# Glaciohound/Chimera-ST

Measured on AMD Instinct MI355X. Metric: train utterances/sec, MuST-C EN-DE s2t_transformer_m, 1/2/4/8 MI355X, higher is better.
Workload: dtype bf16

## Files before the change

chimera-st_amd/csrc/layernorm.hip:

```cpp
#include "cst_common.h"

namespace {

constexpr int LN_MAXV = 4;
constexpr int LN_WAVES = 4;

template <typename T> struct Raw8;
template <> struct Raw8<bf16_t> {
  u32x4 r;
  __device__ __forceinline__ void load(const bf16_t* p) { r = *reinterpret_cast<const u32x4*>(p); }
  __device__ __forceinline__ void unpack(float (&v)[8]) const {
#pragma unroll
    for (int i = 0; i < 4; ++i) { v[2 * i] = __uint_as_float(r[i] << 16); v[2 * i + 1] = __uint_as_float(r[i] & 0xffff0000u); }
  }
};
template <> struct Raw8<float> {
  float f[8];
  __device__ __forceinline__ void load(const float* p) { load8(p, f); }
  __device__ __forceinline__ void unpack(float (&v)[8]) const {
#pragma unroll
    for (int i = 0; i < 8; ++i) v[i] = f[i];
  }
};

// ... 54 lines not shown
#pragma unroll
    for (int i = 0; i < NV; ++i)
      if (lane + 64 * i < nvec) {
#pragma unroll
        for (int e = 0; e < 8; ++e) { const float d = v[i][e] - mu; q += d * d; }
      }
    const float rs = rsqrtf(wave_sum(q) / (float)cols + eps);
#pragma unroll
    for (int i = 0; i < NV; ++i) {
      const int vi = lane + 64 * i;
      if (vi < nvec) {
        float g[8], b[8], o[8];
        gq[i].unpack(g);
        bq[i].unpack(b);
#pragma unroll
        for (int e = 0; e < 8; ++e) o[e] = (v[i][e] - mu) * rs * g[e] + b[e];
        store8(y + row * cols + vi * 8, o);
      }
    }
    if (lane == 0) { mean[row] = mu; rstd[row] = rs; }
  }
}

template <typename T, int NV>
__global__ __launch_bounds__(LN_WAVES * 64, (NV <= 2 ? 4 : 2)) void ln_bwd_kernel(const T* dy, const T* s, const T* gamma, const float* mean,
                                                              const float* rstd, const T* dres, T* dx, float* part,
                                                              int64_t rows, int cols, uint32_t* tile_live, uint32_t epoch) {
  __shared__ float red[LN_WAVES][64 * 8];
  const int lane = threadIdx.x & 63, wave = threadIdx.x >> 6;
  const int nvec = cols / 8;
  float dg[NV][8], db[NV][8], gm[NV][8];
#pragma unroll
  for (int i = 0; i < NV; ++i) {
#pragma unroll
    for (int e = 0; e < 8; ++e) { dg[i][e] = 0.0f; db[i][e] = 0.0f; gm[i][e] = 0.0f; }
    if (lane + 64 * i < nvec) load8(gamma + (lane + 64 * i) * 8, gm[i]);
  }
  for (int64_t row = (int64_t)blockIdx.x * LN_WAVES + wave; row < rows; row += (int64_t)gridDim.x * LN_WAVES) {
    const float mu = mean[row], rs = rstd[row];
    Raw8<T> rd[NV], rx[NV];
    float s1 = 0.0f, s2 = 0.0f;
#pragma unroll
    for (int i = 0; i < NV; ++i) {
      const int vi = lane + 64 * i;
      if (vi < nvec) {
        rd[i].load(dy + row * cols + vi * 8);
        rx[i].load(s + row * cols + vi * 8);
        float d[8], xs[8];
        rd[i].unpack(d);
        rx[i].unpack(xs);
#pragma unroll
        for (int e = 0; e < 8; ++e) {
          const float xh = (xs[e] - mu) * rs;
          const float g = d[e] * gm[i][e];
          s1 += g;
          s2 += g * xh;
          dg[i][e] += d[e] * xh;
          db[i][e] += d[e];
        }
      }
    }
    s1 = wave_sum(s1) / (float)cols;
    s2 = wave_sum(s2) / (float)cols;
    bool nz = false;
#pragma unroll
    for (int i = 0; i < NV; ++i) {
      const int vi = lane + 64 * i;
      if (vi < nvec) {
        float d[8], xs[8], o[8];
        rd[i].unpack(d);
        rx[i].unpack(xs);
#pragma unroll
        for (int e = 0; e < 8; ++e) o[e] = rs * (d[e] * gm[i][e] - s1 - (xs[e] - mu) * rs * s2);
        if (dres) {
          float r[8];
          load8(dres + row * cols + vi * 8, r);
#pragma unroll
          for (int e = 0; e < 8; ++e) o[e] += r[e];
        }
#pragma unroll
        for (int e = 0; e < 8; ++e) nz |= (o[e] != 0.0f);
        store8(dx + row * cols + vi * 8, o);
      }
    }
    if (tile_live && __builtin_amdgcn_ballot_w64(nz) != 0 && lane == 0) tile_live[row >> 6] = epoch;
  }
  float* pg = part + (int64_t)blockIdx.x * 2 * cols;
  float* pb = pg + cols;
#pragma unroll
  for (int i = 0; i < NV; ++i) {
    for (int pass = 0; pass < 2; ++pass) {
      __syncthreads();
#pragma unroll
      for (int e = 0; e < 8; ++e) red[wave][lane * 8 + e] = pass ? db[i][e] : dg[i][e];
      __syncthreads();
      if (wave == 0 && lane + 64 * i < nvec) {
#pragma unroll
        for (int e = 0; e < 8; ++e) {
          float a = 0.0f;
#pragma unroll
          for (int w = 0; w < LN_WAVES; ++w) a += red[w][lane * 8 + e];
          (pass ? pb : pg)[(lane + 64 * i) * 8 + e] = a;
        }
      }
    }
  }
}

template <typename TO>
__global__ __launch_bounds__(1024) void ln_bwd_reduce_kernel(const float* part, TO* dgamma, TO* dbeta, int nblocks, int cols) {
  __shared__ float ra[64][17], rb[64][17];
  const int cl = threadIdx.x & 15, g = threadIdx.x >> 4;
  const int c = blockIdx.x * 16 + cl;
  float a = 0.0f, b = 0.0f;
  if (c < cols)
    for (int i = g; i < nblocks; i += 64) {
      a += part[(int64_t)i * 2 * cols + c];
      b += part[(int64_t)i * 2 * cols + cols + c];
    }
  ra[g][cl] = a;
  rb[g][cl] = b;
  __syncthreads();
  if (g == 0 && c < cols) {
#pragma unroll 8
    for (int k = 1; k < 64; ++k) { a += ra[k][cl]; b += rb[k][cl]; }
    DT<TO>::st(dgamma + c, a);
    DT<TO>::st(dbeta + c, b);
  }
}

int ln_blocks(int64_t rows, int cap = 1024) {
  int64_t b = cst_ceil_div(rows, LN_WAVES);
  return (int)(b < cap ? b : cap);
}
inline int ln_nv(int64_t cols) { return cols <= 512 ? 1 : (cols <= 1024 ? 2 : 4); }

}

extern "C" int cst_layernorm_fwd(const void* x, const void* res, const void* gamma, const void* beta, void* y,
                                 void* sum_out, float* mean, float* rstd, int64_t rows, int64_t cols, float eps,
                                 int dtype, cst_stream stream) {
  CST_REQUIRE(x && gamma && beta && y && mean && rstd, "cst_layernorm_fwd: null tensor");
  CST_REQUIRE(rows > 0 && cols > 0 && cols % 8 == 0 && cols <= 8 * 64 * LN_MAXV, "cst_layernorm_fwd: cols=%lld must be a multiple of 8 and <= %d", (long long)cols, 8 * 64 * LN_MAXV);
  hipStream_t s = (hipStream_t)stream;
  const double bytes = (double)rows * cols * cst_dtype_size(dtype) * (2.0 + (res ? 1.0 : 0.0) + (sum_out ? 1.0 : 0.0));
  CstProfScope prof(CST_K_LAYERNORM, s, 0.0, bytes);
  dim3 grid(ln_blocks(rows, 2048));
  CST_REQUIRE(dtype == CST_BF16 || dtype == CST_F32, "cst_layernorm_fwd: bad dtype %d", dtype);
#define CST_LNF(T, NVV) hipLaunchKernelGGL((ln_fwd_kernel<T, NVV>), grid, dim3(LN_WAVES * 64), 0, s, (const T*)x, (const T*)res, (const T*)gamma, (const T*)beta, (T*)y, (T*)sum_out, mean, rstd, rows, (int)cols, eps)
#define CST_LNF_NV(T) do { const int nv = ln_nv(cols); if (nv == 1) CST_LNF(T, 1); else if (nv == 2) CST_LNF(T, 2); else CST_LNF(T, 4); } while (0)
  if (dtype == CST_BF16) CST_LNF_NV(bf16_t);
  else CST_LNF_NV(float);
#undef CST_LNF_NV
#undef CST_LNF
  return cst_check_launch("cst_layernorm_fwd");
}

constexpr int LN_BWD_BLOCKS = 1024;
extern "C" int64_t cst_layernorm_bwd_workspace(int64_t rows, int64_t cols) {
  return (int64_t)ln_blocks(rows, LN_BWD_BLOCKS) * 2 * cols * (int64_t)sizeof(float);
}

static int layernorm_bwd_impl(const void* dy, const void* sx, const void* gamma, const float* mean, const float* rstd,
                              const void* dres, void* dx, void* dgamma, void* dbeta, void* workspace, int64_t rows,
                              int64_t cols, int dtype, int grad_dtype, uint32_t* tile_live, uint32_t epoch, cst_stream stream) {
  CST_REQUIRE(dy && sx && gamma && mean && rstd && dx && workspace && ((dgamma != nullptr) == (dbeta != nullptr)), "cst_layernorm_bwd: null tensor");
  CST_REQUIRE(rows > 0 && cols > 0 && cols % 8 == 0 && cols <= 8 * 64 * LN_MAXV, "cst_layernorm_bwd: cols=%lld must be a multiple of 8 and <= %d", (long long)cols, 8 * 64 * LN_MAXV);
  hipStream_t s = (hipStream_t)stream;
  const double bytes = (double)rows * cols * cst_dtype_size(dtype) * (3.0 + (dres ? 1.0 : 0.0));
  CstProfScope prof(CST_K_LAYERNORM, s, 0.0, bytes);
  const int nb = ln_blocks(rows, LN_BWD_BLOCKS);
  CST_REQUIRE(dtype == CST_BF16 || dtype == CST_F32, "cst_layernorm_bwd: bad dtype %d", dtype);
#define CST_LNB(T, NVV) hipLaunchKernelGGL((ln_bwd_kernel<T, NVV>), dim3(nb), dim3(LN_WAVES * 64), 0, s, (const T*)dy, (const T*)sx, (const T*)gamma, mean, rstd, (const T*)dres, (T*)dx, (float*)workspace, rows, (int)cols, tile_live, epoch)
#define CST_LNB_NV(T) do { const int nv = ln_nv(cols); if (nv == 1) CST_LNB(T, 1); else if (nv == 2) CST_LNB(T, 2); else CST_LNB(T, 4); } while (0)
  if (dtype == CST_BF16) CST_LNB_NV(bf16_t);
  else CST_LNB_NV(float);
#undef CST_LNB_NV
#undef CST_LNB
  int rc = cst_check_launch("cst_layernorm_bwd");
  if (rc != CST_OK) return rc;
  CST_REQUIRE(grad_dtype == CST_F32 || grad_dtype == dtype, "cst_layernorm_bwd: grad_dtype must be f32 or dtype");
  if (!dgamma) return rc;
  if (grad_dtype == CST_BF16)
    hipLaunchKernelGGL(ln_bwd_reduce_kernel<bf16_t>, dim3((unsigned)cst_ceil_div(cols, 16)), dim3(1024), 0, s, (const float*)workspace, (bf16_t*)dgamma, (bf16_t*)dbeta, nb, (int)cols);
  else
    hipLaunchKernelGGL(ln_bwd_reduce_kernel<float>, dim3((unsigned)cst_ceil_div(cols, 16)), dim3(1024), 0, s, (const float*)workspace, (float*)dgamma, (float*)dbeta, nb, (int)cols);
  return cst_check_launch("cst_layernorm_bwd reduce");
}

extern "C" int cst_layernorm_bwd(const void* dy, const void* sx, const void* gamma, const float* mean, const float* rstd,
                                 const void* dres, void* dx, void* dgamma, void* dbeta, void* workspace, int64_t rows,
                                 int64_t cols, int dtype, int grad_dtype, cst_stream stream) {
  return layernorm_bwd_impl(dy, sx, gamma, mean, rstd, dres, dx, dgamma, dbeta, workspace, rows, cols, dtype, grad_dtype, nullptr, 0, stream);
}

extern "C" int cst_layernorm_bwd_tiles(const void* dy, const void* sx, const void* gamma, const float* mean, const float* rstd,
                                       const void* dres, void* dx, void* dgamma, void* dbeta, void* workspace, int64_t rows,
                                       int64_t cols, int dtype, int grad_dtype, uint32_t* tile_live, uint32_t epoch, cst_stream stream) {
  CST_REQUIRE(tile_live && epoch != 0, "cst_layernorm_bwd_tiles: tile_live / non-zero epoch required");
  return layernorm_bwd_impl(dy, sx, gamma, mean, rstd, dres, dx, dgamma, dbeta, workspace, rows, cols, dtype, grad_dtype, tile_live, epoch, stream);
}
```

chimera-st_amd/functional.py:

```python
import os as _os
import weakref as _weakref

import torch

from . import kernels as K
from . import lib as L

_ACT = {None: L.ACT_NONE, "none": L.ACT_NONE, "relu": L.ACT_RELU, "gelu": L.ACT_GELU}


def _flat2d(x):
    return x.reshape(-1, x.shape[-1]).contiguous()


def _vec(dtype):
    return 8 if dtype == torch.bfloat16 else 4


def _with_tiles(t, tiles):
    if t.is_contiguous():
        t._cst_live_tiles = (tiles[0], tiles[1], t.data_ptr(), t.numel(), t.shape[-1], t._version)
        if t._base is not None:
            t._base._cst_live_tiles = t._cst_live_tiles
    return t


def _tiles_of(t, rows):
    lt = getattr(t, "_cst_live_tiles", None)
    if lt is None and t._base is not None:
        lt = getattr(t._base, "_cst_live_tiles", None)
    if (lt is None or not t.is_contiguous() or lt[2] != t.data_ptr() or lt[3] != t.numel() or lt[4] != t.shape[-1]
            or lt[5] != t._version or lt[0].numel() != (rows + 63) // 64):
        return None
    return (lt[0], lt[1])


_WT_MIN_ROWS = int(_os.environ.get("CST_WT_MIN_ROWS", 512))


def _want_wt(M, w):
    return (M >= _WT_MIN_ROWS and w.is_cuda and w.dim() == 2 and w.is_contiguous() and w.shape[0] % _vec(w.dtype) == 0
            and w.shape[1] % _vec(w.dtype) == 0 and not _os.environ.get("CST_NO_WT"))


def _wversion(w):
    parts = getattr(w, "_cst_parts", None)
    return w._version if parts is None else sum(p._version for p in parts)


class _WeightTransposes:

    def __init__(self):
        self.entries = {}
        self.tables = {}
        self.refreshes = 0
        self.persistent = {}

# ... 125 lines not shown

def _dx_gemm(dz, w, M, *, use_wt, like, resid=None, dact=L.ACT_NONE, aux_in=None, drop=(0.0, 0), m_live=None):
    n_out, n_in = w.shape
    dx = torch.empty(M, n_in, dtype=like.dtype, device=like.device)
    b, b_kmajor, ldb = (WEIGHT_TRANSPOSES.get(w), 1, n_out) if use_wt else (w, 0, n_in)
    K.gemm(dz, b, dx, M, n_in, n_out, a_kmajor=1, b_kmajor=b_kmajor, lda=n_out, ldb=ldb, ldc=n_in, dact=dact, aux_in=aux_in, ld_aux_in=n_in,
           resid=resid, ld_resid=n_in, split_k=1, drop_p=drop[0], drop_key=drop[1], m_live=m_live)
    return dx


def _dw_gemm(dz, x2, w, bias_obj, M, *, db_in_dw, live, dz_travels_on, allow_slot=True, allow_defer=True):
    n_out, n_in = w.shape
    dw = _grad_out(w) if allow_slot else None
    if dw is None:
        dw = torch.empty(n_out, n_in, dtype=w.dtype, device=w.device)
    db = torch.empty(n_out, dtype=w.dtype, device=w.device) if db_in_dw else None
    may = allow_defer and _may_defer(w, bias_obj if db_in_dw else None)
    big = not may or not K.dw_colsum_is_fused(n_out, n_in, M, w.dtype) or dz_travels_on
    K.side_gemm(big, (dz, x2, live[0] if live is not None else None), dz, x2, dw, n_out, n_in, M, a_kmajor=0, b_kmajor=0, lda=n_out, ldb=n_in,
                ldc=n_in, split_k=-1, k_live=live, colsum=db, defer=may)
    return dw, db


def _drop_grad(dy2, drop, out_dtype, live, *, with_colsum, defer):
    if with_colsum and not _os.environ.get("CST_NO_DROP_COLSUM"):
        return K.dropout_colsum(dy2.contiguous(), drop[0], drop[1], out_dtype, live, defer=defer)
    return K.dropout(dy2.contiguous(), *drop), None


def _linear_backward(ctx, dy, dxp):
    x2, w, z = ctx.saved_tensors
    M, Kd = x2.shape
    Np, N = w.shape[0], ctx.N
    if dy is None:
        return dxp, None, None, None, None, None, None
    dy2 = _flat2d(dy)
    live = _tiles_of(dy, M)
    if Np != N:
        dyp = torch.zeros(M, Np, dtype=dy2.dtype, device=dy2.device)
        dyp[:, :N] = dy2
        dy2 = dyp
    db_fused = None
    want_db = ctx.has_bias and ctx.needs_input_grad[2]
    db_in_dw = want_db and ctx.needs_input_grad[1] and Np % 8 == 0 and not _os.environ.get("CST_NO_GEMM_COLSUM") and K.dw_colsum_is_fused(Np, Kd, M, w.dtype)
    may_b = want_db and Np == N and _may_defer(w, ctx.bias_obj)
    if ctx.drop[0] > 0.0:
        dy2, db_fused = _drop_grad(dy2, ctx.drop, w.dtype, live, defer=may_b,
                                   with_colsum=not db_in_dw and ctx.act == L.ACT_NONE and want_db and Np == N and N % 8 == 0)
    dz = K.act_bwd(dy2, z, ctx.act) if ctx.act != L.ACT_NONE else dy2
    dx = dw = db = dres = None
    if ctx.needs_input_grad[0]:
        dx = _dx_gemm(dz, w, M, use_wt=_want_wt(M, w), like=x2, resid=_flat2d(dxp) if dxp is not None else None,
                      m_live=live).view(ctx.xshape)
        if live is not None and dxp is None:
            dx = _with_tiles(dx, live)
    if ctx.needs_input_grad[1]:
        dw, db = _dw_gemm(dz, x2, w, ctx.bias_obj, M, db_in_dw=db_in_dw, live=live, dz_travels_on=dz.data_ptr() == dy.data_ptr() and ctx.has_resid,
                          allow_slot=Np == N, allow_defer=Np == N)
        dw = dw[:N]
        if db is not None:
            db = db[:N]
    if want_db and db is None:
        db = db_fused if db_fused is not None else K.colsum(dz, w.dtype, live, defer=may_b)[:N]
    if ctx.has_resid and ctx.needs_input_grad[3]:
        dres = dy
    return dx, dw, db, dres, None, None, None


class _LinearPassFn(torch.autograd.Function):

    @staticmethod
    def forward(ctx, x, weight, bias, act, drop_p, drop_key):
        y = _LinearFn.forward(ctx, x, weight, bias, None, act, drop_p, drop_key)
        ctx.set_materialize_grads(False)
        return y, x.view_as(x)

    @staticmethod
    def backward(ctx, dy, dxp):
        g = _linear_backward(ctx, dy, dxp)
        return g[0], g[1], g[2], None, None, None


def linear_pass(x, weight, bias=None, act=None, dropout_p=0.0):
    return _LinearPassFn.apply(x, weight, bias, _ACT[act], *_drop_args(dropout_p))


def linear(x, weight, bias=None, act=None, resid=None, dropout_p=0.0):
    return _LinearFn.apply(x, weight, bias, resid, _ACT[act], *_drop_args(dropout_p))


class _FFNFn(torch.autograd.Function):

    @staticmethod
    def forward(ctx, x, w1, b1, w2, b2, resid, act, p_act, key_act, p_out, key_out):
        x2 = _flat2d(x)
        M, d = x2.shape
        F_ = w1.shape[0]
        dout = w2.shape[0]
        z1 = torch.empty(M, F_, dtype=x.dtype, device=x.device)
        h = torch.empty_like(z1)
        K.gemm(x2, w1, h, M, F_, d, a_kmajor=1, b_kmajor=1, lda=d, ldb=d, ldc=F_, bias=b1, act=act, aux_out=z1, ld_aux_out=F_, split_k=1,
               drop_p=p_act, drop_key=key_act)
        y = torch.empty(M, dout, dtype=x.dtype, device=x.device)
        r2 = _flat2d(resid) if resid is not None else None
        K.gemm(h, w2, y, M, dout, F_, a_kmajor=1, b_kmajor=1, lda=F_, ldb=F_, ldc=dout, bias=b2, resid=r2, ld_resid=dout, split_k=1,
               drop_p=p_out, drop_key=key_out)
        ctx.save_for_backward(x2, w1, w2, z1, h)
        ctx.cfg = (act, b1 is not None, b2 is not None, resid is not None, x.shape)
        ctx.res_is_x = (resid is not None and resid.data_ptr() == x.data_ptr() and resid.shape == x.shape
                        and resid.stride() == x.stride() and dout == d)
        ctx.drop = (p_act, key_act, p_out, key_out)
        ctx.bias_objs = (b1, b2)
        return y.view(*x.shape[:-1], dout)

    @staticmethod
    def backward(ctx, dy):
        x2, w1, w2, z1, h = ctx.saved_tensors
        act, has_b1, has_b2, has_res, xshape = ctx.cfg
        M, d = x2.shape
        F_, dout = w1.shape[0], w2.shape[0]
        dy2 = _flat2d(dy)
        live = _tiles_of(dy, M)
        p_act, key_act, p_out, key_out = ctx.drop
        b1, b2 = ctx.bias_objs
        db2_fused = None
        gcs = not _os.environ.get("CST_NO_GEMM_COLSUM")
        db2_in_dw = gcs and has_b2 and ctx.needs_input_grad[4] and ctx.needs_input_grad[3] and dout % 8 == 0 and K.dw_colsum_is_fused(dout, F_, M, w2.dtype)
        db1_in_dw = gcs and has_b1 and ctx.needs_input_grad[2] and ctx.needs_input_grad[1] and F_ % 8 == 0 and K.dw_colsum_is_fused(F_, d, M, w1.dtype)
        if p_out > 0.0:
            dy2, db2_fused = _drop_grad(dy2, (p_out, key_out), w2.dtype, live, defer=_may_defer(w2, b2),
                                        with_colsum=not db2_in_dw and has_b2 and ctx.needs_input_grad[4] and dout % 8 == 0)
        use_wt = _want_wt(M, w2) and _want_wt(M, w1)
        dz1 = _dx_gemm(dy2, w2, M, use_wt=use_wt, like=dy2, dact=act, aux_in=z1, drop=(p_act, key_act), m_live=live)
        dx = dw1 = db1 = dw2 = db2 = None
        if ctx.needs_input_grad[3]:
            dw2, db2 = _dw_gemm(dy2, h, w2, b2, M, db_in_dw=db2_in_dw, live=live, dz_travels_on=dy2.data_ptr() == dy.data_ptr() and has_res)
        if has_b2 and ctx.needs_input_grad[4] and db2 is None:
            db2 = db2_fused if db2_fused is not None else K.colsum(dy2, w2.dtype, live, defer=_may_defer(w2, b2))
        if ctx.needs_input_grad[0]:
            dx = _dx_gemm(dz1, w1, M, use_wt=use_wt, like=x2, resid=_flat2d(dy) if ctx.res_is_x else None, m_live=live).view(xshape)
        if ctx.needs_input_grad[1]:
            dw1, db1 = _dw_gemm(dz1, x2, w1, b1, M, db_in_dw=db1_in_dw, live=live, dz_travels_on=False)
        if has_b1 and ctx.needs_input_grad[2] and db1 is None:
            db1 = K.colsum(dz1, w1.dtype, live, defer=_may_defer(w1, b1))
        dres = dy if has_res and ctx.needs_input_grad[5] and not (ctx.res_is_x and ctx.needs_input_grad[0]) else None
        return dx, dw1, db1, dw2, db2, dres, None, None, None, None, None


def ffn(x, w1, b1, w2, b2, act, resid=None, activation_dropout_p=0.0, dropout_p=0.0):
    assert _ACT[act] != L.ACT_NONE
    return _FFNFn.apply(x, w1.contiguous(), b1, w2.contiguous(), b2, resid, _ACT[act], *_drop_args(activation_dropout_p), *_drop_args(dropout_p))


class _LayerNormFn(torch.autograd.Function):
    @staticmethod
    def forward(ctx, x, res, gamma, beta, eps):
        x2 = _flat2d(x)
        r2 = _flat2d(res) if res is not None else None
        y, s, mean, rstd = K.layernorm_fwd(x2, r2, gamma, beta, eps, want_sum=True)
        src = s if res is not None else x2
        ctx.save_for_backward(src, gamma, mean, rstd)
        ctx.has_res = res is not None
        ctx.shape = x.shape
        ctx.set_materialize_grads(False)
        if res is not None:
            return y.view(x.shape), s.view(x.shape)
        return y.view(x.shape), None

    @staticmethod
    def backward(ctx, dy, ds):
        src, gamma, mean, rstd = ctx.saved_tensors
        if dy is None:
            return ds, (ds if ctx.has_res else None), None, None, None
        dy2 = _flat2d(dy)
        dres = _flat2d(ds) if ds is not None else None
        dx, dg, db, tiles = K.layernorm_bwd(dy2, src, gamma, mean, rstd, dres, grad_dtype=gamma.dtype, want_tiles=True, defer=_may_defer(gamma))
        dx = _with_tiles(dx.view(ctx.shape), tiles)
        return dx, (dx if ctx.has_res else None), dg, db, None


def layer_norm(x, gamma, beta, eps=1e-5):
    return _LayerNormFn.apply(x, None, gamma, beta, eps)[0]


def add_layer_norm(x, res, gamma, beta, eps=1e-5):
    return _LayerNormFn.apply(x, res, gamma, beta, eps)


class _LayerNormPassFn(torch.autograd.Function):

    @staticmethod
    def forward(ctx, x, gamma, beta, eps):
        x2 = _flat2d(x)
        y, _, mean, rstd = K.layernorm_fwd(x2, None, gamma, beta, eps)
        ctx.save_for_backward(x2, gamma, mean, rstd)
        ctx.shape = x.shape
        ctx.set_materialize_grads(False)
        return y.view(x.shape), x.view_as(x)

    @staticmethod
    def backward(ctx, dy, dxp):
        x2, gamma, mean, rstd = ctx.saved_tensors
        dres = _flat2d(dxp) if dxp is not None else None
        if dy is None:
            return (dxp, None, None, None)
        dx, dg, db = K.layernorm_bwd(_flat2d(dy), x2, gamma, mean, rstd, dres, grad_dtype=gamma.dtype, defer=_may_defer(gamma))
        return dx.view(ctx.shape), dg, db, None


def layer_norm_residual(x, gamma, beta, eps=1e-5):
    return _LayerNormPassFn.apply(x, gamma, beta, eps)


_MASK_CACHE = []


_PAD_TILES = []


def _pad_tiles(u8):
    for src, pt in _PAD_TILES:
        if src is u8:
            return pt
    flat = u8.reshape(-1)
    pad = (-flat.numel()) % 64
    if pad:
        flat = torch.cat([flat, torch.ones(pad, dtype=flat.dtype, device=flat.device)])
    pt = flat.view(-1, 64).amin(dim=1) > 0
    _PAD_TILES.append((u8, pt))
    if len(_PAD_TILES) > 8:
# ... 667 lines not shown
```

chimera-st_amd/kernels.py:

```python
import ctypes
import os

import torch

from . import lib as L

_ws = {}
STATS = {}


def workspace(nbytes: int, device) -> torch.Tensor:
    key = (device.index, L.stream_ptr().value)
    t = _ws.get(key)
    if t is None or t.numel() < nbytes:
        t = torch.empty(max(nbytes, 1 << 20), dtype=torch.uint8, device=device)
        _ws[key] = t
    return t


class _Deferred:

    MAX_BYTES = 32 << 20

    def __init__(self):
# ... 232 lines not shown
def layernorm_bwd(dy, s, gamma, mean, rstd, dres=None, grad_dtype=torch.float32, want_tiles=False, defer=False):
    dy, s = _2d(dy), _2d(s)
    rows, cols = s.shape
    lib = L.load()
    dx = torch.empty_like(s)
    dg = torch.empty(cols, dtype=grad_dtype, device=s.device)
    db = torch.empty(cols, dtype=grad_dtype, device=s.device)
    stamps, epoch = (torch.empty((rows + 63) // 64, dtype=torch.int32, device=s.device), next_epoch()) if want_tiles else (None, 0)

    def launch(ws, pg, pb):
        if want_tiles:
            L.check(lib.cst_layernorm_bwd_tiles(L.ptr(dy), L.ptr(s), L.ptr(gamma), L.ptr(mean), L.ptr(rstd), L.ptr(dres), L.ptr(dx), pg,
                                                pb, L.ptr(ws), rows, cols, L.dtype_code(s.dtype), L.dtype_code(grad_dtype),
                                                L.ptr(stamps), epoch, L.stream_ptr()), "cst_layernorm_bwd_tiles")
        else:
            L.check(lib.cst_layernorm_bwd(L.ptr(dy), L.ptr(s), L.ptr(gamma), L.ptr(mean), L.ptr(rstd), L.ptr(dres), L.ptr(dx), pg,
                                          pb, L.ptr(ws), rows, cols, L.dtype_code(s.dtype), L.dtype_code(grad_dtype), L.stream_ptr()),
                    "cst_layernorm_bwd")

    _two_stage(lib.cst_layernorm_bwd_workspace(rows, cols), (dg, db), defer, launch)
    return (dx, dg, db, (stamps, epoch)) if want_tiles else (dx, dg, db)


def _bhtd_strides(t, layout):
    assert t.stride(-1) == 1
    if layout == "bt":
        return t.stride(0), None, t.stride(1)
    return t.stride(1), None, t.stride(0)


def attn_desc(q, k, v, o, lse, H, D, kpm, causal, scale, layout_q="bt", layout_kv="bt", drop_p=0.0, drop_key=0, kv_len=None, seq=None):
    d = L.AttnDesc()
    d.dtype = L.dtype_code(q.dtype)
    if layout_q == "bt":
        B, Tq = q.shape[0], q.shape[1]
    else:
        Tq, B = q.shape[0], q.shape[1]
    Tk = k.shape[1] if layout_kv == "bt" else k.shape[0]
    if seq is not None:
        assert layout_q == "bt" and layout_kv == "bt" and B == 1 and kpm is None
        assert seq[0].dtype == torch.int32 and seq[0].is_contiguous()
        B, Tq, Tk = seq[0].numel() - 1, int(seq[1]), int(seq[1])
        d.seq_offsets = seq[0].data_ptr()
        STATS["attn_packed"] = STATS.get("attn_packed", 0) + 1
    else:
        d.seq_offsets = None
# ... 468 lines not shown
```

chimera-st_amd/lib.py:

```python
import ctypes
import os

import torch

_HERE = os.path.dirname(os.path.abspath(__file__))
LIB_PATH = os.path.join(_HERE, "libcst_hip.so")
ABI_VERSION = 10

F32, BF16 = 0, 1
ACT_NONE, ACT_RELU, ACT_GELU = 0, 1, 2
BIAS_NONE, BIAS_COL, BIAS_ROW = 0, 1, 2
K_GEMM, K_ATTN_FWD, K_ATTN_BWD, K_LAYERNORM, K_CONV0, K_ELEMENTWISE, K_LOSS, K_OPTIM = range(8)
KERNEL_CLASSES = ["gemm", "attn_fwd", "attn_bwd", "layernorm", "conv0", "elementwise", "loss", "optim"]

c_i64, c_int, c_f, c_p = ctypes.c_int64, ctypes.c_int, ctypes.c_float, ctypes.c_void_p


class GemmDesc(ctypes.Structure):
    _fields_ = [
        ("dtype", c_int), ("c_dtype", c_int), ("a_kmajor", c_int), ("b_kmajor", c_int),
        ("M", c_i64), ("N", c_i64), ("K", c_i64),
        ("A", c_p), ("lda", c_i64), ("a_seg", c_i64), ("a_seg_stride", c_i64),
        ("B", c_p), ("ldb", c_i64), ("b_seg", c_i64), ("b_seg_stride", c_i64),
        ("C", c_p), ("ldc", c_i64),
        ("bias", c_p), ("bias_mode", c_int), ("sbias0", c_i64), ("sbias1", c_i64),
        ("act", c_int),
        ("aux_out", c_p), ("ld_aux_out", c_i64),
        ("dact", c_int),
        ("aux_in", c_p), ("ld_aux_in", c_i64),
        ("resid", c_p), ("ld_resid", c_i64),
# ... 65 lines not shown
        ("B", c_i64), ("S", c_i64), ("T", c_i64),
        ("wave", c_p), ("n_samples", c_p), ("out", c_p), ("n_frames", c_p),
        ("utterance_cmvn", c_int), ("norm_means", c_int), ("norm_vars", c_int),
        ("global_mean", c_p), ("global_std", c_p),
        ("global_first", c_int),
        ("specaugment", c_int),
        ("n_fmask", c_int), ("n_tmask", c_int),
        ("fmask", c_p), ("tmask", c_p),
        ("mask_mean", c_int), ("mask_value", c_f),
        ("workspace", c_p), ("workspace_bytes", c_i64),
    ]


SYMBOLS = [
    ("cst_last_error", ctypes.c_char_p, []),
    ("cst_version", c_int, []),
    ("cst_device_arch_ok", c_int, []),
    ("cst_prof_enable", None, [c_int]),
    ("cst_prof_query", c_i64, [c_int, ctypes.POINTER(ctypes.c_double), ctypes.POINTER(ctypes.c_double), ctypes.POINTER(ctypes.c_double)]),
    ("cst_layernorm_fwd", c_int, [c_p, c_p, c_p, c_p, c_p, c_p, c_p, c_p, c_i64, c_i64, c_f, c_int, c_p]),
    ("cst_layernorm_bwd_workspace", c_i64, [c_i64, c_i64]),
    ("cst_layernorm_bwd", c_int, [c_p, c_p, c_p, c_p, c_p, c_p, c_p, c_p, c_p, c_p, c_i64, c_i64, c_int, c_int, c_p]),
    ("cst_layernorm_bwd_tiles", c_int, [c_p, c_p, c_p, c_p, c_p, c_p, c_p, c_p, c_p, c_p, c_i64, c_i64, c_int, c_int, c_p, ctypes.c_uint32, c_p]),
    ("cst_gemm_workspace", c_i64, [ctypes.POINTER(GemmDesc)]),
    ("cst_gemm_colsum_is_fused", c_int, [ctypes.POINTER(GemmDesc)]),
    ("cst_gemm_splits", c_int, [ctypes.POINTER(GemmDesc)]),
    ("cst_reduce_multi", c_int, [ctypes.POINTER(ReduceItem), c_int, c_p]),
    ("cst_gemm", c_int, [ctypes.POINTER(GemmDesc), c_p]),
    ("cst_prof_dump", c_i64, [c_int, ctypes.c_char_p, c_i64]),
    ("cst_gemm_reserve_cus", c_int, [c_int]),
    ("cst_transpose2d", c_int, [c_p, c_p, c_i64, c_i64, c_int, c_p]),
    ("cst_transpose2d_multi", c_int, [c_p, c_int, c_i64, c_int, c_p]),
    ("cst_weight_norm_workspace", c_i64, [c_i64, c_i64]),
    ("cst_weight_norm_fwd", c_int, [c_p, c_p, c_p, c_p, c_p, c_i64, c_i64, c_int, c_p]),
    ("cst_weight_norm_bwd", c_int, [c_p, c_p, c_p, c_p, c_p, c_p, c_p, c_i64, c_i64, c_int, c_p]),
    ("cst_attn_bwd_workspace", c_i64, [ctypes.POINTER(AttnDesc)]),
    ("cst_attn_fwd", c_int, [ctypes.POINTER(AttnDesc), c_p]),
    ("cst_attn_bwd", c_int, [ctypes.POINTER(AttnDesc), c_p]),
    ("cst_conv0_fwd_workspace", c_i64, [c_i64, c_i64, c_int, c_int]),
    ("cst_conv0_gn_gelu_fwd", c_int, [c_p, c_p, c_p, c_p, c_p, c_p, c_p, c_p, c_p, c_p, c_i64, c_i64, c_i64, c_int, c_int, c_f, c_int, c_p]),
    ("cst_conv0_bwd_workspace", c_i64, [c_i64, c_i64, c_i64, c_int, c_int]),
    ("cst_conv0_gn_gelu_bwd", c_int, [c_p, c_p, c_p, c_p, c_p, c_p, c_p, c_p, c_p, c_p, c_p, c_p, c_p, c_i64, c_i64, c_i64, c_int, c_int, c_int, c_p]),
    ("cst_conv0_ln_gelu_fwd", c_int, [c_p, c_p, c_p, c_p, c_p, c_p, c_p, c_p, c_p, c_i64, c_i64, c_i64, c_int, c_int, c_f, c_int, c_p]),
    ("cst_conv0_ln_bwd_workspace", c_i64, [c_i64, c_i64, c_i64, c_int, c_int]),
    ("cst_conv0_ln_gelu_bwd", c_int, [c_p, c_p, c_p, c_p, c_p, c_p, c_p, c_p, c_p, c_p, c_p, c_p, c_p, c_p, c_i64, c_i64, c_i64, c_int, c_int, c_int, c_p]),
    ("cst_ln_gelu_fwd", c_int, [c_p, c_p, c_p, c_p, c_p, c_p, c_p, c_i64, c_i64, c_i64, c_f, c_int, c_p]),
# ... 124 lines not shown
```

include/cst.h:

```cpp
#ifndef CST_H
#define CST_H

#include <stdint.h>

#ifdef __cplusplus
extern "C" {
#endif

#define CST_ABI_VERSION 10

typedef enum { CST_F32 = 0, CST_BF16 = 1 } cst_dtype;

typedef enum {
  CST_OK = 0,
  CST_ERR_BAD_ARG = -1,
  CST_ERR_LAUNCH = -2,
  CST_ERR_WORKSPACE = -3,
  CST_ERR_UNSUPPORTED = -4
} cst_status;

typedef void* cst_stream;

const char* cst_last_error(void);
int cst_version(void);
int cst_device_arch_ok(void);

typedef enum {
  CST_K_GEMM = 0, CST_K_ATTN_FWD, CST_K_ATTN_BWD, CST_K_LAYERNORM, CST_K_CONV0, CST_K_ELEMENTWISE,
  CST_K_LOSS, CST_K_OPTIM, CST_K_NUM
} cst_kernel_class;
void cst_prof_enable(int on);
int64_t cst_prof_query(int kernel_class, double* total_ms, double* flops, double* bytes);
int64_t cst_prof_dump(int kernel_class, char* buf, int64_t cap);

int cst_layernorm_fwd(const void* x, const void* res, const void* gamma, const void* beta,
                      void* y, void* sum_out, float* mean, float* rstd,
                      int64_t rows, int64_t cols, float eps, int dtype, cst_stream stream);
int64_t cst_layernorm_bwd_workspace(int64_t rows, int64_t cols);
int cst_layernorm_bwd(const void* dy, const void* s, const void* gamma, const float* mean,
                      const float* rstd, const void* dres, void* dx, void* dgamma, void* dbeta,
                      void* workspace, int64_t rows, int64_t cols, int dtype, int grad_dtype, cst_stream stream);
int cst_layernorm_bwd_tiles(const void* dy, const void* s, const void* gamma, const float* mean,
                            const float* rstd, const void* dres, void* dx, void* dgamma, void* dbeta,
                            void* workspace, int64_t rows, int64_t cols, int dtype, int grad_dtype,
                            uint32_t* tile_live, uint32_t epoch, cst_stream stream);

typedef enum { CST_ACT_NONE = 0, CST_ACT_RELU = 1, CST_ACT_GELU = 2 } cst_act;
typedef enum { CST_BIAS_NONE = 0, CST_BIAS_COL = 1, CST_BIAS_ROW = 2 } cst_bias_mode;

typedef struct {
  int dtype;
  int c_dtype;
  int a_kmajor, b_kmajor;
  int64_t M, N, K;
  const void* A; int64_t lda, a_seg, a_seg_stride;
  const void* B; int64_t ldb, b_seg, b_seg_stride;
  void* C; int64_t ldc;
  const void* bias; int bias_mode;
  int64_t sbias0, sbias1;
  int act;
  void* aux_out; int64_t ld_aux_out;
  int dact;
  const void* aux_in; int64_t ld_aux_in;
  const void* resid; int64_t ld_resid;
  float alpha;
  float drop_p; uint32_t drop_key;
  int64_t batch0, batch1;
  int64_t sa0, sa1, sb0, sb1, sc0, sc1;
// ... 211 lines not shown
```

Before: 520.1.

## Fuse dropout-mask backward and bias colsum into LayerNorm backward kernel

The LayerNorm backward kernel now applies the downstream dropout mask to dx and writes a masked copy. It can also accumulate the column sum of that masked gradient as the preceding linear layer's bias gradient, using shared memory and an extra workspace slab. Python glue tags linear/FFN outputs with their dropout parameters so the later dropout-backward pass reuses the masked gradient instead of launching a separate dropout or dropout-colsum kernel over dy. This removes one full read/write pass per residual block, in exchange for an extra store in the LN kernel, more shared memory, and fragile tensor-attribute matching.

```diff
diff --git a/chimera-st_amd/csrc/layernorm.hip b/chimera-st_amd/csrc/layernorm.hip
--- a/chimera-st_amd/csrc/layernorm.hip
+++ b/chimera-st_amd/csrc/layernorm.hip
@@ -100,11 +100,29 @@
   }
 }
 
-template <typename T, int NV>
-__global__ __launch_bounds__(LN_WAVES * 64, (NV <= 2 ? 4 : 2)) void ln_bwd_kernel(const T* dy, const T* s, const T* gamma, const float* mean,
-                                                              const float* rstd, const T* dres, T* dx, float* part,
-                                                              int64_t rows, int cols, uint32_t* tile_live, uint32_t epoch) {
+__device__ __forceinline__ void store8_rounded(bf16_t* p, float (&v)[8]) {
+  bf16x8 r;
+#pragma unroll
+  for (int i = 0; i < 8; ++i) r[i] = static_cast<__bf16>(v[i]);
+  *reinterpret_cast<bf16x8*>(p) = r;
+#pragma unroll
+  for (int i = 0; i < 8; ++i) v[i] = static_cast<float>(r[i]);
+}
+__device__ __forceinline__ void store8_rounded(float* p, float (&v)[8]) {
+  store8(p, v);
+#pragma unroll
+  for (int i = 0; i < 8; ++i) asm volatile("" : "+v"(v[i]));
+}
+
+template <typename T> struct LnDropArgs { T* dxm; uint32_t key, thr; float scale; };
+
+template <typename T, int NV, int DROP>
+__device__ __forceinline__ void ln_bwd_body(const T* dy, const T* s, const T* gamma, const float* mean,
+                                            const float* rstd, const T* dres, T* dx, float* part,
+                                            int64_t rows, int cols, uint32_t* tile_live, uint32_t epoch,
+                                            const LnDropArgs<T>& dr) {
   __shared__ float red[LN_WAVES][64 * 8];
+  __shared__ f32x4 dcs[DROP == 2 ? LN_WAVES * NV * 2 * 64 : 1];
   const int lane = threadIdx.x & 63, wave = threadIdx.x >> 6;
   const int nvec = cols / 8;
   float dg[NV][8], db[NV][8], gm[NV][8];
@@ -113,6 +131,11 @@
 #pragma unroll
     for (int e = 0; e < 8; ++e) { dg[i][e] = 0.0f; db[i][e] = 0.0f; gm[i][e] = 0.0f; }
     if (lane + 64 * i < nvec) load8(gamma + (lane + 64 * i) * 8, gm[i]);
+  }
+  if constexpr (DROP == 2) {
+    const f32x4 z = {0.0f, 0.0f, 0.0f, 0.0f};
+#pragma unroll
+    for (int i = 0; i < NV * 2; ++i) dcs[(wave * NV * 2 + i) * 64 + lane] = z;
   }
   for (int64_t row = (int64_t)blockIdx.x * LN_WAVES + wave; row < rows; row += (int64_t)gridDim.x * LN_WAVES) {
     const float mu = mean[row], rs = rstd[row];
@@ -158,12 +181,28 @@
         }
 #pragma unroll
         for (int e = 0; e < 8; ++e) nz |= (o[e] != 0.0f);
-        store8(dx + row * cols + vi * 8, o);
+        if constexpr (DROP != 0) {
+          store8_rounded(dx + row * cols + vi * 8, o);
+          cst_drop8(o, dr.key, (uint64_t)(row * cols + vi * 8), dr.thr, dr.scale);
+          if constexpr (DROP == 2) {
+            store8_rounded(dr.dxm + row * cols + vi * 8, o);
+            f32x4* slot = dcs + (wave * NV * 2 + i * 2) * 64 + lane;
+            f32x4 a = slot[0], b = slot[64];
+#pragma unroll
+            for (int e = 0; e < 4; ++e) { a[e] += o[e]; b[e] += o[4 + e]; }
+            slot[0] = a;
+            slot[64] = b;
+          } else {
+            store8(dr.dxm + row * cols + vi * 8, o);
+          }
+        } else {
+          store8(dx + row * cols + vi * 8, o);
+        }
       }
     }
     if (tile_live && __builtin_amdgcn_ballot_w64(nz) != 0 && lane == 0) tile_live[row >> 6] = epoch;
   }
-  float* pg = part + (int64_t)blockIdx.x * 2 * cols;
+  float* pg = part + (int64_t)blockIdx.x * (DROP == 2 ? 3 : 2) * cols;
   float* pb = pg + cols;
 #pragma unroll
   for (int i = 0; i < NV; ++i) {
@@ -183,27 +222,60 @@
       }
     }
   }
+  if constexpr (DROP == 2) {
+    __syncthreads();
+#pragma unroll
+    for (int i = 0; i < NV; ++i) {
+      if (wave == 0 && lane + 64 * i < nvec) {
+#pragma unroll
+        for (int h = 0; h < 2; ++h) {
+          f32x4 a = {0.0f, 0.0f, 0.0f, 0.0f};
+#pragma unroll
+          for (int w = 0; w < LN_WAVES; ++w) a += dcs[(w * NV * 2 + i * 2 + h) * 64 + lane];
+          *reinterpret_cast<f32x4*>(pb + cols + (lane + 64 * i) * 8 + h * 4) = a;
+        }
+      }
+    }
+  }
+}
+
+template <typename T, int NV>
+__global__ __launch_bounds__(LN_WAVES * 64, (NV <= 2 ? 4 : 2)) void ln_bwd_kernel(const T* dy, const T* s, const T* gamma, const float* mean,
+                                                              const float* rstd, const T* dres, T* dx, float* part,
+                                                              int64_t rows, int cols, uint32_t* tile_live, uint32_t epoch) {
+  ln_bwd_body<T, NV, 0>(dy, s, gamma, mean, rstd, dres, dx, part, rows, cols, tile_live, epoch, LnDropArgs<T>{});
+}
+template <typename T, int NV, int DROP>
+__global__ __launch_bounds__(LN_WAVES * 64, (NV <= 2 ? 4 : 2)) void ln_bwd_kernel_drop(const T* dy, const T* s, const T* gamma, const float* mean,
+                                                              const float* rstd, const T* dres, T* dx, float* part,
+                                                              int64_t rows, int cols, uint32_t* tile_live, uint32_t epoch,
+                                                              LnDropArgs<T> dr) {
+  ln_bwd_body<T, NV, DROP>(dy, s, gamma, mean, rstd, dres, dx, part, rows, cols, tile_live, epoch, dr);
 }
 
 template <typename TO>
-__global__ __launch_bounds__(1024) void ln_bwd_reduce_kernel(const float* part, TO* dgamma, TO* dbeta, int nblocks, int cols) {
-  __shared__ float ra[64][17], rb[64][17];
+__global__ __launch_bounds__(1024) void ln_bwd_reduce_kernel(const float* part, TO* dgamma, TO* dbeta, int nblocks, int cols, TO* dbias) {
+  __shared__ float ra[64][17], rb[64][17], rc[64][17];
   const int cl = threadIdx.x & 15, g = threadIdx.x >> 4;
   const int c = blockIdx.x * 16 + cl;
-  float a = 0.0f, b = 0.0f;
+  const int np = dbias ? 3 : 2;
+  float a = 0.0f, b = 0.0f, d = 0.0f;
   if (c < cols)
     for (int i = g; i < nblocks; i += 64) {
-      a += part[(int64_t)i * 2 * cols + c];
-      b += part[(int64_t)i * 2 * cols + cols + c];
+      a += part[(int64_t)i * np * cols + c];
+      b += part[(int64_t)i * np * cols + cols + c];
+      if (dbias) d += part[(int64_t)i * np * cols + 2 * cols + c];
     }
   ra[g][cl] = a;
   rb[g][cl] = b;
+  rc[g][cl] = d;
   __syncthreads();
   if (g == 0 && c < cols) {
 #pragma unroll 8
-    for (int k = 1; k < 64; ++k) { a += ra[k][cl]; b += rb[k][cl]; }
+    for (int k = 1; k < 64; ++k) { a += ra[k][cl]; b += rb[k][cl]; d += rc[k][cl]; }
     DT<TO>::st(dgamma + c, a);
     DT<TO>::st(dbeta + c, b);
+    if (dbias) DT<TO>::st(dbias + c, d);
   }
 }
 
@@ -241,28 +313,36 @@
 
 static int layernorm_bwd_impl(const void* dy, const void* sx, const void* gamma, const float* mean, const float* rstd,
                               const void* dres, void* dx, void* dgamma, void* dbeta, void* workspace, int64_t rows,
-                              int64_t cols, int dtype, int grad_dtype, uint32_t* tile_live, uint32_t epoch, cst_stream stream) {
+                              int64_t cols, int dtype, int grad_dtype, uint32_t* tile_live, uint32_t epoch, cst_stream stream,
+                              void* dxm = nullptr, void* dbias = nullptr, float drop_p = 0.0f, uint32_t drop_key = 0) {
   CST_REQUIRE(dy && sx && gamma && mean && rstd && dx && workspace && ((dgamma != nullptr) == (dbeta != nullptr)), "cst_layernorm_bwd: null tensor");
   CST_REQUIRE(rows > 0 && cols > 0 && cols % 8 == 0 && cols <= 8 * 64 * LN_MAXV, "cst_layernorm_bwd: cols=%lld must be a multiple of 8 and <= %d", (long long)cols, 8 * 64 * LN_MAXV);
   hipStream_t s = (hipStream_t)stream;
-  const double bytes = (double)rows * cols * cst_dtype_size(dtype) * (3.0 + (dres ? 1.0 : 0.0));
+  const double bytes = (double)rows * cols * cst_dtype_size(dtype) * (3.0 + (dres ? 1.0 : 0.0) + (dxm ? 1.0 : 0.0));
   CstProfScope prof(CST_K_LAYERNORM, s, 0.0, bytes);
   const int nb = ln_blocks(rows, LN_BWD_BLOCKS);
   CST_REQUIRE(dtype == CST_BF16 || dtype == CST_F32, "cst_layernorm_bwd: bad dtype %d", dtype);
-#define CST_LNB(T, NVV) hipLaunchKernelGGL((ln_bwd_kernel<T, NVV>), dim3(nb), dim3(LN_WAVES * 64), 0, s, (const T*)dy, (const T*)sx, (const T*)gamma, mean, rstd, (const T*)dres, (T*)dx, (float*)workspace, rows, (int)cols, tile_live, epoch)
-#define CST_LNB_NV(T) do { const int nv = ln_nv(cols); if (nv == 1) CST_LNB(T, 1); else if (nv == 2) CST_LNB(T, 2); else CST_LNB(T, 4); } while (0)
+  const int drop = dxm ? (dbias ? 2 : 1) : 0;
+  const uint32_t thr = drop ? cst_drop_thr16(drop_p) : 0u;
+  const float scale = drop ? 1.0f / (1.0f - drop_p) : 1.0f;
+#define CST_LNB_ARGS(T) dim3(nb), dim3(LN_WAVES * 64), 0, s, (const T*)dy, (const T*)sx, (const T*)gamma, mean, rstd, (const T*)dres, (T*)dx, (float*)workspace, rows, (int)cols, tile_live, epoch
+#define CST_LNB(T, NVV, DR) hipLaunchKernelGGL((ln_bwd_kernel_drop<T, NVV, DR>), CST_LNB_ARGS(T), LnDropArgs<T>{(T*)dxm, drop_key, thr, scale})
+#define CST_LNB_DR(T, NVV) do { if (drop == 0) hipLaunchKernelGGL((ln_bwd_kernel<T, NVV>), CST_LNB_ARGS(T)); else if (drop == 1) CST_LNB(T, NVV, 1); else CST_LNB(T, NVV, 2); } while (0)
+#define CST_LNB_NV(T) do { const int nv = ln_nv(cols); if (nv == 1) CST_LNB_DR(T, 1); else if (nv == 2) CST_LNB_DR(T, 2); else CST_LNB_DR(T, 4); } while (0)
   if (dtype == CST_BF16) CST_LNB_NV(bf16_t);
   else CST_LNB_NV(float);
 #undef CST_LNB_NV
+#undef CST_LNB_DR
+#undef CST_LNB_ARGS
 #undef CST_LNB
   int rc = cst_check_launch("cst_layernorm_bwd");
   if (rc != CST_OK) return rc;
   CST_REQUIRE(grad_dtype == CST_F32 || grad_dtype == dtype, "cst_layernorm_bwd: grad_dtype must be f32 or dtype");
   if (!dgamma) return rc;
   if (grad_dtype == CST_BF16)
-    hipLaunchKernelGGL(ln_bwd_reduce_kernel<bf16_t>, dim3((unsigned)cst_ceil_div(cols, 16)), dim3(1024), 0, s, (const float*)workspace, (bf16_t*)dgamma, (bf16_t*)dbeta, nb, (int)cols);
+    hipLaunchKernelGGL(ln_bwd_reduce_kernel<bf16_t>, dim3((unsigned)cst_ceil_div(cols, 16)), dim3(1024), 0, s, (const float*)workspace, (bf16_t*)dgamma, (bf16_t*)dbeta, nb, (int)cols, (bf16_t*)dbias);
   else
-    hipLaunchKernelGGL(ln_bwd_reduce_kernel<float>, dim3((unsigned)cst_ceil_div(cols, 16)), dim3(1024), 0, s, (const float*)workspace, (float*)dgamma, (float*)dbeta, nb, (int)cols);
+    hipLaunchKernelGGL(ln_bwd_reduce_kernel<float>, dim3((unsigned)cst_ceil_div(cols, 16)), dim3(1024), 0, s, (const float*)workspace, (float*)dgamma, (float*)dbeta, nb, (int)cols, (float*)dbias);
   return cst_check_launch("cst_layernorm_bwd reduce");
 }
 
@@ -270,6 +350,21 @@
                                  const void* dres, void* dx, void* dgamma, void* dbeta, void* workspace, int64_t rows,
                                  int64_t cols, int dtype, int grad_dtype, cst_stream stream) {
   return layernorm_bwd_impl(dy, sx, gamma, mean, rstd, dres, dx, dgamma, dbeta, workspace, rows, cols, dtype, grad_dtype, nullptr, 0, stream);
+}
+
+extern "C" int64_t cst_layernorm_bwd_drop_workspace(int64_t rows, int64_t cols, int with_dbias) {
+  return (int64_t)ln_blocks(rows, LN_BWD_BLOCKS) * (with_dbias ? 3 : 2) * cols * (int64_t)sizeof(float);
+}
+
+extern "C" int cst_layernorm_bwd_drop(const void* dy, const void* sx, const void* gamma, const float* mean, const float* rstd,
+                                      const void* dres, void* dx, void* dgamma, void* dbeta, void* workspace, int64_t rows,
+                                      int64_t cols, int dtype, int grad_dtype, uint32_t* tile_live, uint32_t epoch, void* dxm,
+                                      void* dbias, float drop_p, uint32_t drop_key, cst_stream stream) {
+  CST_REQUIRE(dxm && dxm != dx, "cst_layernorm_bwd_drop: dxm required, distinct from dx");
+  CST_REQUIRE(drop_p > 0.0f && drop_p < 1.0f, "cst_layernorm_bwd_drop: drop_p must be in (0, 1)");
+  CST_REQUIRE(!tile_live || epoch != 0, "cst_layernorm_bwd_drop: stamps need a non-zero epoch");
+  return layernorm_bwd_impl(dy, sx, gamma, mean, rstd, dres, dx, dgamma, dbeta, workspace, rows, cols, dtype, grad_dtype, tile_live, epoch, stream,
+                            dxm, dbias, drop_p, drop_key);
 }
 
 extern "C" int cst_layernorm_bwd_tiles(const void* dy, const void* sx, const void* gamma, const float* mean, const float* rstd,
diff --git a/chimera-st_amd/functional.py b/chimera-st_amd/functional.py
--- a/chimera-st_amd/functional.py
+++ b/chimera-st_amd/functional.py
@@ -33,6 +33,53 @@
             or lt[5] != t._version or lt[0].numel() != (rows + 63) // 64):
         return None
     return (lt[0], lt[1])
+
+
+def _mark_grad_drop(y, p, key, want_db, want_dw, w, bias_obj, k_in, plain):
+    if y.is_contiguous():
+        y._cst_grad_drop = (p, key, want_db, want_dw, w, bias_obj, k_in, plain, y.data_ptr(), y.numel(), y.shape[-1], y._version)
+        if y._base is not None:
+            y._base._cst_grad_drop = y._cst_grad_drop
+    return y
+
+
+def _attr_of(t, name):
+    m = getattr(t, name, None)
+    if m is None and t._base is not None:
+        m = getattr(t._base, name, None)
+    if m is None or not t.is_contiguous() or m[-4] != t.data_ptr() or m[-3] != t.numel() or m[-2] != t.shape[-1] or m[-1] != t._version:
+        return None
+    return m
+
+
+def _grad_drop_of(x):
+    m = _attr_of(x, "_cst_grad_drop")
+    return None if m is None else m[:8]
+
+
+def _with_dxm(dx, dxm, dbias, p, key):
+    dx._cst_dxm = (p, key, dxm, [dbias], dx.data_ptr(), dx.numel(), dx.shape[-1], dx._version)
+    if dx._base is not None:
+        dx._base._cst_dxm = dx._cst_dxm
+    return dx
+
+
+def _db_route(want_db, want_dw, n_out, k_in, M, dtype, plain):
+    db_in_dw = bool(want_db and want_dw and n_out % 8 == 0 and not _os.environ.get("CST_NO_GEMM_COLSUM") and K.dw_colsum_is_fused(n_out, k_in, M, dtype))
+    return db_in_dw, bool(want_db and not db_in_dw and plain and n_out % 8 == 0)
+
+
+def _ln_bwd(dy2, src, gamma, mean, rstd, dres, gd, want_tiles):
+    if gd is None or _os.environ.get("CST_NO_LN_DROP"):
+        r = K.layernorm_bwd(dy2, src, gamma, mean, rstd, dres, grad_dtype=gamma.dtype, want_tiles=want_tiles, defer=_may_defer(gamma))
+        return r[0], r[1], r[2], (r[3] if want_tiles else None), None
+    p, key, want_db, want_dw, w, bias_obj, k_in, plain = gd
+    want_bias = (_db_route(want_db, want_dw, w.shape[0], k_in, src.shape[0], w.dtype, plain)[1] and w.dtype == gamma.dtype
+                 and not _os.environ.get("CST_NO_DROP_COLSUM"))
+    defer = _may_defer(gamma) and (not want_bias or _may_defer(w, bias_obj))
+    dx, dg, db, dxm, dbias, tiles = K.layernorm_bwd_drop(dy2, src, gamma, mean, rstd, p, key, dres, grad_dtype=gamma.dtype,
+                                                         want_tiles=want_tiles, want_bias=want_bias, defer=defer)
+    return dx, dg, db, tiles, (dxm, dbias, p, key)
 
 
 _WT_MIN_ROWS = int(_os.environ.get("CST_WT_MIN_ROWS", 512))
@@ -204,8 +251,15 @@
     return dw, db
 
 
-def _drop_grad(dy2, drop, out_dtype, live, *, with_colsum, defer):
-    if with_colsum and not _os.environ.get("CST_NO_DROP_COLSUM"):
+def _drop_grad(dy2, drop, out_dtype, live, *, with_colsum, defer, src=None):
+    with_colsum = with_colsum and not _os.environ.get("CST_NO_DROP_COLSUM")
+    m = _attr_of(src, "_cst_dxm") if src is not None and not _os.environ.get("CST_NO_LN_DROP") else None
+    if m is not None and m[0] == drop[0] and m[1] == drop[1] and m[2].shape == dy2.shape:
+        if not with_colsum:
+            return m[2], None
+        if m[3] and m[3][0] is not None and m[3][0].dtype == out_dtype:
+            return m[2], m[3].pop()
+    if with_colsum:
         return K.dropout_colsum(dy2.contiguous(), drop[0], drop[1], out_dtype, live, defer=defer)
     return K.dropout(dy2.contiguous(), *drop), None
 
@@ -224,11 +278,10 @@
         dy2 = dyp
     db_fused = None
     want_db = ctx.has_bias and ctx.needs_input_grad[2]
-    db_in_dw = want_db and ctx.needs_input_grad[1] and Np % 8 == 0 and not _os.environ.get("CST_NO_GEMM_COLSUM") and K.dw_colsum_is_fused(Np, Kd, M, w.dtype)
+    db_in_dw, with_colsum = _db_route(want_db, ctx.needs_input_grad[1], Np, Kd, M, w.dtype, ctx.act == L.ACT_NONE and Np == N)
     may_b = want_db and Np == N and _may_defer(w, ctx.bias_obj)
     if ctx.drop[0] > 0.0:
-        dy2, db_fused = _drop_grad(dy2, ctx.drop, w.dtype, live, defer=may_b,
-                                   with_colsum=not db_in_dw and ctx.act == L.ACT_NONE and want_db and Np == N and N % 8 == 0)
+        dy2, db_fused = _drop_grad(dy2, ctx.drop, w.dtype, live, defer=may_b, with_colsum=with_colsum, src=dy if Np == N else None)
     dz = K.act_bwd(dy2, z, ctx.act) if ctx.act != L.ACT_NONE else dy2
     dx = dw = db = dres = None
     if ctx.needs_input_grad[0]:
@@ -268,7 +321,12 @@
 
 
 def linear(x, weight, bias=None, act=None, resid=None, dropout_p=0.0):
-    return _LinearFn.apply(x, weight, bias, resid, _ACT[act], *_drop_args(dropout_p))
+    p, key = _drop_args(dropout_p)
+    y = _LinearFn.apply(x, weight, bias, resid, _ACT[act], p, key)
+    if p > 0.0 and torch.is_grad_enabled() and weight.shape[0] % _vec(x.dtype) == 0:
+        _mark_grad_drop(y, p, key, bias is not None and bias.requires_grad, weight.requires_grad, weight, bias, weight.shape[1],
+                        _ACT[act] == L.ACT_NONE)
+    return y
 
 
 class _FFNFn(torch.autograd.Function):
@@ -307,11 +365,10 @@
         b1, b2 = ctx.bias_objs
         db2_fused = None
         gcs = not _os.environ.get("CST_NO_GEMM_COLSUM")
-        db2_in_dw = gcs and has_b2 and ctx.needs_input_grad[4] and ctx.needs_input_grad[3] and dout % 8 == 0 and K.dw_colsum_is_fused(dout, F_, M, w2.dtype)
+        db2_in_dw, db2_colsum = _db_route(has_b2 and ctx.needs_input_grad[4], ctx.needs_input_grad[3], dout, F_, M, w2.dtype, True)
         db1_in_dw = gcs and has_b1 and ctx.needs_input_grad[2] and ctx.needs_input_grad[1] and F_ % 8 == 0 and K.dw_colsum_is_fused(F_, d, M, w1.dtype)
         if p_out > 0.0:
-            dy2, db2_fused = _drop_grad(dy2, (p_out, key_out), w2.dtype, live, defer=_may_defer(w2, b2),
-                                        with_colsum=not db2_in_dw and has_b2 and ctx.needs_input_grad[4] and dout % 8 == 0)
+            dy2, db2_fused = _drop_grad(dy2, (p_out, key_out), w2.dtype, live, defer=_may_defer(w2, b2), with_colsum=db2_colsum, src=dy)
         use_wt = _want_wt(M, w2) and _want_wt(M, w1)
         dz1 = _dx_gemm(dy2, w2, M, use_wt=use_wt, like=dy2, dact=act, aux_in=z1, drop=(p_act, key_act), m_live=live)
         dx = dw1 = db1 = dw2 = db2 = None
@@ -331,7 +388,12 @@
 
 def ffn(x, w1, b1, w2, b2, act, resid=None, activation_dropout_p=0.0, dropout_p=0.0):
     assert _ACT[act] != L.ACT_NONE
-    return _FFNFn.apply(x, w1.contiguous(), b1, w2.contiguous(), b2, resid, _ACT[act], *_drop_args(activation_dropout_p), *_drop_args(dropout_p))
+    p_act, key_act = _drop_args(activation_dropout_p)
+    p, key = _drop_args(dropout_p)
+    y = _FFNFn.apply(x, w1.contiguous(), b1, w2.contiguous(), b2, resid, _ACT[act], p_act, key_act, p, key)
+    if p > 0.0 and torch.is_grad_enabled():
+        _mark_grad_drop(y, p, key, b2 is not None and b2.requires_grad, w2.requires_grad, w2, b2, w2.shape[1], True)
+    return y
 
 
 class _LayerNormFn(torch.autograd.Function):
@@ -344,6 +406,7 @@
         ctx.save_for_backward(src, gamma, mean, rstd)
         ctx.has_res = res is not None
         ctx.shape = x.shape
+        ctx.grad_drop = _grad_drop_of(x)
         ctx.set_materialize_grads(False)
         if res is not None:
             return y.view(x.shape), s.view(x.shape)
@@ -356,8 +419,10 @@
             return ds, (ds if ctx.has_res else None), None, None, None
         dy2 = _flat2d(dy)
         dres = _flat2d(ds) if ds is not None else None
-        dx, dg, db, tiles = K.layernorm_bwd(dy2, src, gamma, mean, rstd, dres, grad_dtype=gamma.dtype, want_tiles=True, defer=_may_defer(gamma))
+        dx, dg, db, tiles, masked = _ln_bwd(dy2, src, gamma, mean, rstd, dres, ctx.grad_drop, True)
         dx = _with_tiles(dx.view(ctx.shape), tiles)
+        if masked is not None:
+            dx = _with_dxm(dx, *masked)
         return dx, (dx if ctx.has_res else None), dg, db, None
 
 
@@ -377,6 +442,7 @@
         y, _, mean, rstd = K.layernorm_fwd(x2, None, gamma, beta, eps)
         ctx.save_for_backward(x2, gamma, mean, rstd)
         ctx.shape = x.shape
+        ctx.grad_drop = _grad_drop_of(x)
         ctx.set_materialize_grads(False)
         return y.view(x.shape), x.view_as(x)
 
@@ -386,8 +452,11 @@
         dres = _flat2d(dxp) if dxp is not None else None
         if dy is None:
             return (dxp, None, None, None)
-        dx, dg, db = K.layernorm_bwd(_flat2d(dy), x2, gamma, mean, rstd, dres, grad_dtype=gamma.dtype, defer=_may_defer(gamma))
-        return dx.view(ctx.shape), dg, db, None
+        dx, dg, db, _, masked = _ln_bwd(_flat2d(dy), x2, gamma, mean, rstd, dres, ctx.grad_drop, False)
+        dx = dx.view(ctx.shape)
+        if masked is not None:
+            dx = _with_dxm(dx, *masked)
+        return dx, dg, db, None
 
 
 def layer_norm_residual(x, gamma, beta, eps=1e-5):
diff --git a/chimera-st_amd/kernels.py b/chimera-st_amd/kernels.py
--- a/chimera-st_amd/kernels.py
+++ b/chimera-st_amd/kernels.py
@@ -278,6 +278,24 @@
     return (dx, dg, db, (stamps, epoch)) if want_tiles else (dx, dg, db)
 
 
+def layernorm_bwd_drop(dy, s, gamma, mean, rstd, p, key, dres=None, grad_dtype=torch.float32, want_tiles=False, want_bias=False, defer=False):
+    dy, s = _2d(dy), _2d(s)
+    rows, cols = s.shape
+    lib = L.load()
+    dx, dxm = torch.empty_like(s), torch.empty_like(s)
+    outs = [torch.empty(cols, dtype=grad_dtype, device=s.device) for _ in range(3 if want_bias else 2)]
+    stamps, epoch = (torch.empty((rows + 63) // 64, dtype=torch.int32, device=s.device), next_epoch()) if want_tiles else (None, 0)
+
+    def launch(ws, pg, pb, pbias=None):
+        L.check(lib.cst_layernorm_bwd_drop(L.ptr(dy), L.ptr(s), L.ptr(gamma), L.ptr(mean), L.ptr(rstd), L.ptr(dres), L.ptr(dx), pg, pb,
+                                           L.ptr(ws), rows, cols, L.dtype_code(s.dtype), L.dtype_code(grad_dtype), L.ptr(stamps), epoch,
+                                           L.ptr(dxm), L.ptr(outs[2]) if want_bias else None, float(p), int(key) & 0xFFFFFFFF, L.stream_ptr()),
+                "cst_layernorm_bwd_drop")
+
+    _two_stage(lib.cst_layernorm_bwd_drop_workspace(rows, cols, int(want_bias)), tuple(outs), defer, launch)
+    return dx, outs[0], outs[1], dxm, (outs[2] if want_bias else None), ((stamps, epoch) if want_tiles else None)
+
+
 def _bhtd_strides(t, layout):
     assert t.stride(-1) == 1
     if layout == "bt":
diff --git a/chimera-st_amd/lib.py b/chimera-st_amd/lib.py
--- a/chimera-st_amd/lib.py
+++ b/chimera-st_amd/lib.py
@@ -5,7 +5,7 @@
 
 _HERE = os.path.dirname(os.path.abspath(__file__))
 LIB_PATH = os.path.join(_HERE, "libcst_hip.so")
-ABI_VERSION = 10
+ABI_VERSION = 11
 
 F32, BF16 = 0, 1
 ACT_NONE, ACT_RELU, ACT_GELU = 0, 1, 2
@@ -117,6 +117,9 @@
     ("cst_layernorm_bwd_workspace", c_i64, [c_i64, c_i64]),
     ("cst_layernorm_bwd", c_int, [c_p, c_p, c_p, c_p, c_p, c_p, c_p, c_p, c_p, c_p, c_i64, c_i64, c_int, c_int, c_p]),
     ("cst_layernorm_bwd_tiles", c_int, [c_p, c_p, c_p, c_p, c_p, c_p, c_p, c_p, c_p, c_p, c_i64, c_i64, c_int, c_int, c_p, ctypes.c_uint32, c_p]),
+    ("cst_layernorm_bwd_drop_workspace", c_i64, [c_i64, c_i64, c_int]),
+    ("cst_layernorm_bwd_drop", c_int, [c_p, c_p, c_p, c_p, c_p, c_p, c_p, c_p, c_p, c_p, c_i64, c_i64, c_int, c_int, c_p, ctypes.c_uint32, c_p, c_p, c_f,
+                                       ctypes.c_uint32, c_p]),
     ("cst_gemm_workspace", c_i64, [ctypes.POINTER(GemmDesc)]),
     ("cst_gemm_colsum_is_fused", c_int, [ctypes.POINTER(GemmDesc)]),
     ("cst_gemm_splits", c_int, [ctypes.POINTER(GemmDesc)]),
diff --git a/include/cst.h b/include/cst.h
--- a/include/cst.h
+++ b/include/cst.h
@@ -7,7 +7,7 @@
 extern "C" {
 #endif
 
-#define CST_ABI_VERSION 10
+#define CST_ABI_VERSION 11
 
 typedef enum { CST_F32 = 0, CST_BF16 = 1 } cst_dtype;
 
@@ -44,6 +44,12 @@
                             const float* rstd, const void* dres, void* dx, void* dgamma, void* dbeta,
                             void* workspace, int64_t rows, int64_t cols, int dtype, int grad_dtype,
                             uint32_t* tile_live, uint32_t epoch, cst_stream stream);
+int64_t cst_layernorm_bwd_drop_workspace(int64_t rows, int64_t cols, int with_dbias);
+int cst_layernorm_bwd_drop(const void* dy, const void* s, const void* gamma, const float* mean,
+                           const float* rstd, const void* dres, void* dx, void* dgamma, void* dbeta,
+                           void* workspace, int64_t rows, int64_t cols, int dtype, int grad_dtype,
+                           uint32_t* tile_live, uint32_t epoch, void* dxm, void* dbias, float drop_p,
+                           uint32_t drop_key, cst_stream stream);
 
 typedef enum { CST_ACT_NONE = 0, CST_ACT_RELU = 1, CST_ACT_GELU = 2 } cst_act;
 typedef enum { CST_BIAS_NONE = 0, CST_BIAS_COL = 1, CST_BIAS_ROW = 2 } cst_bias_mode;
```

Result: no change. 519.1 (-0.2%).
